# Ced3-han/PepFlowww

Hardware: AMD Instinct MI355X
Metric: residues x denoise-steps / s (higher is better)
Workload: dtype f32 (fp32 storage and accumulation; matrix products as 3 x f16 split MFMA, ~22-bit operands); 1 GPU; cfg4/GPU: B=64 x 128-residue synthetic pockets (112 ctx + 16 gen) per GPU; per_gpu_batch=64, residues=128, global_batch=64, parallelism=batch-shard x1, hipgraph=True, precision=fp32

## Files before the change

### pepflowww_amd/csrc/ipa_split.hip

```cpp
#include <cstdlib>
#include <type_traits>
#include "common.h"
#include "../../include/pepflow_hip.h"

#ifdef PF_PROFILE
__device__ long long g_prof_ipas[64];
#define PROFS(i) do { if (blockIdx.x == gridDim.x / 2 + 3 && threadIdx.x == 64) g_prof_ipas[i] = clock64(); } while (0)
extern "C" int pf_debug_prof_ipas(long long* out, int n) {
    return (int)hipMemcpyFromSymbol(out, HIP_SYMBOL(g_prof_ipas), sizeof(long long) * n, 0, hipMemcpyDeviceToHost);
}
#else
#define PROFS(i)
#endif

namespace {

typedef float f32x2 __attribute__((ext_vector_type(2)));
constexpr int H = PF_HEADS, C = PF_C_HID, PQ = PF_QK_PTS, PV = PF_V_PTS;
constexpr int OFF_KV = 1024;
#ifndef PF_IPA_WMAX
#define PF_IPA_WMAX 8
#endif
constexpr int WMAX = PF_IPA_WMAX;
constexpr int KPS = 28;
// ... 968 lines not shown
        }
    };
    half8 kh[4], nh[4];
    if constexpr (!PROJ) { if (wave_on) loadk(0, kh); }

    if constexpr (PROJ) {
        for (int j = tid; j < LK; j += blockDim.x) MJ[j] = a.mask[rowb + j];
        for (int idx = tid; idx < PF_ATT_VROWS * (L32 - LK); idx += blockDim.x) {
            const int row = idx / (L32 - LK), col = LK + idx - row * (L32 - LK);
            VT[row * VTS + col] = (_Float16)0.f;
        }
        unsigned char* WS = reinterpret_cast<unsigned char*>(SW);
        float* QPW = reinterpret_cast<float*>(WS + PJ16_STAGE_B) + wave * (1536 / 4);
        float* PB = reinterpret_cast<float*>(WS + PJ16_STAGE_B) + (blockDim.x >> 6) * (1536 / 4);
        proj_head16<KF>(a, rowb, wave_on ? iq : 0, h, i0 + r, wave_on, KP, KL, VT, VTS, WS, QPW, PB, qh, qp4, lane, wave, (int)(blockDim.x >> 6));
        __syncthreads();
        if (!wave_on) return;
        loadk(0, kh);
    } else {

    {
        const int nth = blockDim.x;
        constexpr int KB = 6;
        float4 k4[KB];
#pragma unroll
        for (int u = 0; u < KB; ++u) {
            const int idx = min(tid + u * nth, max(LK * 6 - 1, 0)), j = idx / 6, q = idx - j * 6;
            k4[u] = *reinterpret_cast<const float4*>(a.kp + (rowb + j) * 192 + h * 24 + 4 * q);
        }
        float mj0 = a.mask[rowb + min(tid, max(LK - 1, 0))];
        asm volatile("" : "+v"(k4[0].x), "+v"(k4[0].y), "+v"(k4[0].z), "+v"(k4[0].w), "+v"(k4[1].x), "+v"(k4[1].y), "+v"(k4[1].z), "+v"(k4[1].w),
                          "+v"(k4[2].x), "+v"(k4[2].y), "+v"(k4[2].z), "+v"(k4[2].w), "+v"(mj0));
        asm volatile("" : "+v"(k4[3].x), "+v"(k4[3].y), "+v"(k4[3].z), "+v"(k4[3].w), "+v"(k4[4].x), "+v"(k4[4].y), "+v"(k4[4].z), "+v"(k4[4].w),
                          "+v"(k4[5].x), "+v"(k4[5].y), "+v"(k4[5].z), "+v"(k4[5].w));
#pragma unroll
        for (int u = 0; u < KB; ++u) {
            const int idx = tid + u * nth, j = idx / 6, q = idx - j * 6;
            if (idx < LK * 6) *reinterpret_cast<float4*>(KP + j * KPS + 4 * q) = k4[u];
        }
        if (tid < LK) MJ[tid] = mj0;
        for (int idx = tid + KB * nth; idx < LK * 6; idx += nth) {
            const int j = idx / 6, q = idx - j * 6;
            *reinterpret_cast<float4*>(KP + j * KPS + 4 * q) = *reinterpret_cast<const float4*>(a.kp + (rowb + j) * 192 + h * 24 + 4 * q);
        }
        for (int j = tid + nth; j < LK; j += nth) MJ[j] = a.mask[rowb + j];
    }
    __syncthreads();
    if (!wave_on) return;
    }
    PROFS(1);

    const float scale_qk = 0.051031036307982884f;
    const float* brow = a.bias + (((size_t)b * H + h) * L + iq) * L;
    float* srow = SW + (size_t)wave * 16 * SLD + r * SLD;
    float mx = -3.0e38f;
    auto qk_tile = [&](int t, const half8 (&kh)[4], const float4& bv) {
        const int jb = 16 * t + 4 * g;
        const float bj[4] = {bv.x, bv.y, bv.z, bv.w};
        f32x4 am = {0.f, 0.f, 0.f, 0.f};
#pragma unroll
        for (int s4 = 0; s4 < 4; ++s4) am = mfma_h(kh[s4], qh[s4], am);
        float sv[4];
#pragma unroll
        for (int e = 0; e < 4; ++e) {
            const int j = jb + e;
            const float* kp = KP + j * KPS;
            f32x2 d2 = {0.f, 0.f};
#pragma unroll
            for (int q = 0; q < 6; ++q) {
                const float4 kq = *reinterpret_cast<const float4*>(kp + 4 * q);
                const f32x2 da = (f32x2){qp4[q].x, qp4[q].y} - (f32x2){kq.x, kq.y};
                const f32x2 db = (f32x2){qp4[q].z, qp4[q].w} - (f32x2){kq.z, kq.w};
                d2 = __builtin_elementwise_fma(da, da, d2);
                d2 = __builtin_elementwise_fma(db, db, d2);
            }
            float v = am[e] * scale_qk + bj[e];
            v = v + (-0.5f) * (gamma * (d2[0] + d2[1]));
            v = v + 1e5f * (mi * MJ[j] - 1.f);
            sv[e] = v;
            mx = fmaxf(mx, v);
        }
        *reinterpret_cast<float4*>(srow + jb) = make_float4(sv[0], sv[1], sv[2], sv[3]);
    };
    {
        float4 bc = *reinterpret_cast<const float4*>(brow + 4 * g), bn;
        int t = 0;
        for (; t + 1 < kt; t += 2) {
            loadk(t + 1, nh);
            bn = *reinterpret_cast<const float4*>(brow + 16 * (t + 1) + 4 * g);
            __builtin_amdgcn_sched_barrier(0);
            qk_tile(t, kh, bc);
            __builtin_amdgcn_sched_barrier(0);
            loadk(min(t + 2, kt - 1), kh);
            bc = *reinterpret_cast<const float4*>(brow + 16 * min(t + 2, kt - 1) + 4 * g);
            __builtin_amdgcn_sched_barrier(0);
            qk_tile(t + 1, nh, bn);
            __builtin_amdgcn_sched_barrier(0);
        }
        if (kt & 1) qk_tile(kt - 1, kh, bc);
    }
    PROFS(2);
    mx = max_xor32(max_xor16(mx));
    float sum = 0.f;
    for (int t = 0; t < kt; ++t) {
        float4 v = *reinterpret_cast<const float4*>(srow + 16 * t + 4 * g);
        v.x = exp_softmax(v.x - mx); v.y = exp_softmax(v.y - mx); v.z = exp_softmax(v.z - mx); v.w = exp_softmax(v.w - mx);
        sum += v.x; sum += v.y; sum += v.z; sum += v.w;
        *reinterpret_cast<float4*>(srow + 16 * t + 4 * g) = v;
    }
    if (L32 > LK) *reinterpret_cast<float4*>(srow + LK + 4 * g) = make_float4(0.f, 0.f, 0.f, 0.f);
    sum = sum_xor32(sum_xor16(sum));
    const float inv = 1.f / sum;
    asm volatile("s_waitcnt lgkmcnt(0)" ::: "memory");
    __builtin_amdgcn_wave_barrier();
    PROFS(3);
    if constexpr (FUSE) pair_dz_phase<true>(a, rowb, h, i0, LK, kt, SW + (size_t)wave * 16 * SLD, SLD, inv, lane);
    PROFS(7);
    float* prow = FUSE ? nullptr : a.p_out + (((size_t)b * H + h) * L + iq) * L;

    constexpr int NTC = 11;
    const _Float16* vt = reinterpret_cast<const _Float16*>(a.att_vt) + ((size_t)b * H + h) * PF_ATT_VT_HEAD(L);
    int vrow[NTC];
#pragma unroll
    for (int n = 0; n < NTC; ++n) vrow[n] = n < 8 ? 8 * r + n : min(128 + 16 * (n - 8) + r, PF_ATT_VROWS - 1);
    auto loadv = [&](int s32, half8 (&vh)[NTC]) {
#pragma unroll
        for (int n = 0; n < NTC; ++n) {
            if constexpr (PROJ) vh[n] = *reinterpret_cast<const half8*>(VT + vrow[n] * VTS + 32 * s32 + 8 * g);
            else vh[n] = *reinterpret_cast<const half8*>(vt + ((size_t)(n * PF_ATT_VT_NST(L) + s32) * 64 + lane) * 8);
        }
    };
    f32x4 Om[NTC];
#pragma unroll
    for (int n = 0; n < NTC; ++n) Om[n] = (f32x4){0.f, 0.f, 0.f, 0.f};
    const int ns = L32 >> 5;
    auto pv_step = [&](int s32, const half8 (&vh)[NTC]) {
        float4 p0 = *reinterpret_cast<const float4*>(srow + 32 * s32 + 8 * g);
        float4 p1 = *reinterpret_cast<const float4*>(srow + 32 * s32 + 8 * g + 4);
        p0.x *= inv; p0.y *= inv; p0.z *= inv; p0.w *= inv;
        p1.x *= inv; p1.y *= inv; p1.z *= inv; p1.w *= inv;
        if (!FUSE && 32 * s32 + 8 * g < LK) {
            *reinterpret_cast<float4*>(prow + 32 * s32 + 8 * g) = p0;
            *reinterpret_cast<float4*>(prow + 32 * s32 + 8 * g + 4) = p1;
        }
        half8 ph;
        ph[0] = (_Float16)p0.x; ph[1] = (_Float16)p0.y; ph[2] = (_Float16)p0.z; ph[3] = (_Float16)p0.w;
        ph[4] = (_Float16)p1.x; ph[5] = (_Float16)p1.y; ph[6] = (_Float16)p1.z; ph[7] = (_Float16)p1.w;
#pragma unroll
        for (int n = 0; n < NTC; ++n) Om[n] = mfma_h(ph, vh[n], Om[n]);
    };
    {
        half8 va[NTC], vb2[NTC];
        loadv(0, va);
        int s32 = 0;
        for (; s32 + 1 < ns; s32 += 2) {
            loadv(s32 + 1, vb2);
            __builtin_amdgcn_sched_barrier(0);
            pv_step(s32, va);
            __builtin_amdgcn_sched_barrier(0);
            loadv(min(s32 + 2, ns - 1), va);
            __builtin_amdgcn_sched_barrier(0);
            pv_step(s32 + 1, vb2);
            __builtin_amdgcn_sched_barrier(0);
        }
        if (ns & 1) pv_step(ns - 1, va);
    }
    PROFS(4);
    float* opt = SW + (size_t)wave * 16 * SLD;
    asm volatile("s_waitcnt lgkmcnt(0)" ::: "memory");
    __builtin_amdgcn_wave_barrier();
#pragma unroll
    for (int e = 0; e < 4; ++e) {
        const int ti = 4 * g + e, i = i0 + ti;
        float o[NTC];
#pragma unroll
        for (int n = 0; n < NTC; ++n) o[n] = Om[n][e];
        float* f = a.feats + (rowb + i) * PF_IPA_FEATS + h * C + 8 * r;
        *reinterpret_cast<float4*>(f) = make_float4(o[0], o[1], o[2], o[3]);
        *reinterpret_cast<float4*>(f + 4) = make_float4(o[4], o[5], o[6], o[7]);
        opt[ti * 36 + r] = o[8];
        opt[ti * 36 + 16 + r] = o[9];
        if (r < 4) opt[ti * 36 + 32 + r] = o[10];
    }
    asm volatile("s_waitcnt lgkmcnt(0)" ::: "memory");
    __builtin_amdgcn_wave_barrier();
    PROFS(5);
    for (int idx = lane; idx < 16 * PV; idx += 64) {
        const int ti = idx / PV, p = idx - ti * PV;
        const int i = i0 + ti;
        const float* R = a.rot + (rowb + i) * 9;
        const float* T = a.trans + (rowb + i) * 3;
        const float* o = opt + ti * 36 + p * 3;
        const float x = o[0] - T[0], y = o[1] - T[1], z = o[2] - T[2];
        const float lx = R[0] * x + R[3] * y + R[6] * z;
        const float ly = R[1] * x + R[4] * y + R[7] * z;
        const float lz = R[2] * x + R[5] * y + R[8] * z;
        float* f = a.feats + (rowb + i) * PF_IPA_FEATS + h * PV + p;
        f[1024] = lx;
        f[1120] = ly;
        f[1216] = lz;
        f[1312] = sqrtf(lx * lx + ly * ly + lz * lz + 1e-8f);
    }
    PROFS(6);
}

constexpr int ZW = 4;
template <int NG, bool Z16 = false>
__global__ __launch_bounds__(64 * ZW) void ipa_pair_kernel(pf_ipa_attn_args a) {
    constexpr int LPZ = 16 * NG;
    extern __shared__ __attribute__((aligned(16))) float smem[];
    const int tid = threadIdx.x, wave = tid >> 6, lane = tid & 63;
    const int r = lane & 15, g = lane >> 4;
    const int L = a.L;
    float* PL = smem;
    float* ZBAR = PL + 8 * LPZ;
    float* WL = ZBAR + ZW * 8 * 64;
    const long row = blockIdx.x;
    const long b = row / L, i = row - b * L;
    const int Le = a.key_end ? min(__builtin_amdgcn_readfirstlane(a.key_end[b]), L) : L;
    if (i >= Le) return;
    const int nge = (Le + 15) >> 4;
    const float* zrow = a.z + (size_t)row * L * 64 + 4 * r;
    const _Float16* zrow16 = reinterpret_cast<const _Float16*>(a.z) + (size_t)row * L * 64 + 4 * r;
    float4 zq[NG];
    half4 zq16[NG];
#pragma unroll
    for (int u = 0; u < NG; ++u) {
        const int j = 4 * (4 * u + wave) + g;
        if (u < nge) {
            if constexpr (Z16) zq16[u] = *reinterpret_cast<const half4*>(zrow16 + (size_t)min(j, L - 1) * 64);
            else zq[u] = *reinterpret_cast<const float4*>(zrow + (size_t)min(j, L - 1) * 64);
        }
    }
    const float4 wq4 = *reinterpret_cast<const float4*>(a.w_dz + r * 64 + 16 * g + 4 * wave);    const float bdz = a.b_dz[r];
    if ((L & 3) == 0) {
        for (int idx = tid; idx < LPZ * 2; idx += 64 * ZW) {
            const int hh = idx / (LPZ / 4), j = 4 * (idx - hh * (LPZ / 4));
            float4 v = make_float4(0.f, 0.f, 0.f, 0.f);
            if (j < Le) {
                v = *reinterpret_cast<const float4*>(a.p_out + ((b * H + hh) * L + i) * L + j);
                if (j + 1 >= Le) v.y = 0.f;
                if (j + 2 >= Le) v.z = 0.f;
                if (j + 3 >= Le) v.w = 0.f;
            }
            *reinterpret_cast<float4*>(PL + hh * LPZ + j) = v;
        }
    } else {
        for (int idx = tid; idx < LPZ * 8; idx += 64 * ZW) {
            const int hh = idx / LPZ, j = idx - hh * LPZ;
            PL[idx] = j < Le ? a.p_out[((b * H + hh) * L + i) * L + j] : 0.f;
        }
    }
    *reinterpret_cast<float4*>(WL + (wave * 64 + lane) * 4) = wq4;
    __syncthreads();
    f32x4 zacc[4];
#pragma unroll
    for (int ct = 0; ct < 4; ++ct) zacc[ct] = (f32x4){0.f, 0.f, 0.f, 0.f};
    const float* pl = PL + (r & 7) * LPZ + g;
    const float keep = r < 8 ? 1.f : 0.f;
#pragma unroll
    for (int u = 0; u < NG; ++u) {
        if (u < nge) {
            const float pa = pl[4 * (4 * u + wave)] * keep;
            if constexpr (Z16) zq[u] = make_float4((float)zq16[u][0], (float)zq16[u][1], (float)zq16[u][2], (float)zq16[u][3]);
            zacc[0] = mfma16(pa, zq[u].x, zacc[0]);
            zacc[1] = mfma16(pa, zq[u].y, zacc[1]);
            zacc[2] = mfma16(pa, zq[u].z, zacc[2]);
            zacc[3] = mfma16(pa, zq[u].w, zacc[3]);
        }
    }
    if (g < 2) {
        float* zb = ZBAR + wave * H * 64;
#pragma unroll
        for (int e = 0; e < 4; ++e)
            *reinterpret_cast<float4*>(zb + (4 * g + e) * 64 + 4 * r) = make_float4(zacc[0][e], zacc[1][e], zacc[2][e], zacc[3][e]);
    }
    __syncthreads();
    if (wave == 0) {
        f32x4 oacc[4];
#pragma unroll
        for (int q = 0; q < 4; ++q) oacc[q] = (f32x4){0.f, 0.f, 0.f, 0.f};
        float wdz[16];
#pragma unroll
        for (int q = 0; q < 4; ++q) {
            const float4 w4 = *reinterpret_cast<const float4*>(WL + (q * 64 + lane) * 4);
            wdz[4 * q] = w4.x; wdz[4 * q + 1] = w4.y; wdz[4 * q + 2] = w4.z; wdz[4 * q + 3] = w4.w;
        }
        const float* zs = ZBAR + (r & 7) * 64 + 16 * g;
#pragma unroll
        for (int s4 = 0; s4 < 16; ++s4) {
            float za = zs[s4];
#pragma unroll
            for (int q = 1; q < ZW; ++q) za += zs[q * H * 64 + s4];
            oacc[s4 & 3] = mfma16(za * keep, wdz[s4], oacc[s4 & 3]);
        }
        if (g < 2) {
#pragma unroll
            for (int e = 0; e < 4; ++e)
                a.feats[(size_t)row * PF_IPA_FEATS + 1408 + (4 * g + e) * 16 + r] = ((oacc[0][e] + oacc[1][e]) + (oacc[2][e] + oacc[3][e])) + bdz;
        }
    }
}

template <int NG, bool D16 = false>
__global__ __launch_bounds__(256) void ipa_pair_dz_kernel(pf_ipa_attn_args a) {
    constexpr int LPZ = 16 * NG;
    extern __shared__ __attribute__((aligned(16))) float smem[];
    const int tid = threadIdx.x, wave = tid >> 6, lane = tid & 63;
    const int r = lane & 15, g = lane >> 4;
    const int L = a.L;
    const long row = (long)blockIdx.x * 4 + wave;
    if (row >= (long)a.B * L) return;
    const long b = row / L, i = row - b * L;
    const int Le = a.key_end ? min(__builtin_amdgcn_readfirstlane(a.key_end[b]), L) : L;
    if (i >= Le) return;
    const int nge = (Le + 15) >> 4;
    float* PL = smem + wave * 8 * LPZ;
    const float* drow = a.dz + (size_t)row * L * 16 + r;
    const _Float16* drow16 = reinterpret_cast<const _Float16*>(a.dz) + (size_t)row * L * 16 + r;
    float bv[NG][4];
    _Float16 bv16[NG][4];
#pragma unroll
    for (int u = 0; u < NG; ++u)
        if (u < nge) {
#pragma unroll
            for (int t = 0; t < 4; ++t) {
                const size_t off = (size_t)min(16 * u + 4 * t + g, L - 1) * 16;
                if constexpr (D16) bv16[u][t] = drow16[off];
                else bv[u][t] = drow[off];
            }
        }
    const float bdz = a.b_dz[r];
    if ((L & 3) == 0) {
        for (int idx = lane; idx < LPZ * 2; idx += 64) {
            const int hh = idx / (LPZ / 4), j = 4 * (idx - hh * (LPZ / 4));
            float4 v = make_float4(0.f, 0.f, 0.f, 0.f);
            if (j < Le) {
                v = *reinterpret_cast<const float4*>(a.p_out + ((b * H + hh) * L + i) * L + j);
                if (j + 1 >= Le) v.y = 0.f;
                if (j + 2 >= Le) v.z = 0.f;
                if (j + 3 >= Le) v.w = 0.f;
            }
            float* d = PL + hh * LPZ + (j & ~15) + ((j >> 2) & 3);
            d[0] = v.x; d[4] = v.y; d[8] = v.z; d[12] = v.w;
        }
    } else {
        for (int idx = lane; idx < LPZ * 8; idx += 64) {
            const int hh = idx / LPZ, j = idx - hh * LPZ;
            PL[hh * LPZ + (j & ~15) + 4 * (j & 3) + ((j >> 2) & 3)] = j < Le ? a.p_out[((b * H + hh) * L + i) * L + j] : 0.f;
        }
    }
    asm volatile("s_waitcnt lgkmcnt(0)" ::: "memory");
    __builtin_amdgcn_wave_barrier();
    f32x4 acc[4];
#pragma unroll
    for (int t = 0; t < 4; ++t) acc[t] = (f32x4){0.f, 0.f, 0.f, 0.f};
    const float* pl = PL + (r & 7) * LPZ + 4 * g;
    const float keep = r < 8 ? 1.f : 0.f;
#pragma unroll
    for (int u = 0; u < NG; ++u) {
        if (u < nge) {
            const float4 pa = *reinterpret_cast<const float4*>(pl + 16 * u);
            if constexpr (D16) {
#pragma unroll
                for (int t = 0; t < 4; ++t) bv[u][t] = (float)bv16[u][t];
            }
            acc[0] = mfma16(pa.x * keep, bv[u][0], acc[0]);
            acc[1] = mfma16(pa.y * keep, bv[u][1], acc[1]);
            acc[2] = mfma16(pa.z * keep, bv[u][2], acc[2]);
            acc[3] = mfma16(pa.w * keep, bv[u][3], acc[3]);
        }
    }
    if (g < 2) {
        float* f = a.feats + (size_t)row * PF_IPA_FEATS + 1408 + r;
#pragma unroll
        for (int e = 0; e < 4; ++e) f[(4 * g + e) * 16] = ((acc[0][e] + acc[1][e]) + (acc[2][e] + acc[3][e])) + bdz;
    }
}

template <int NG>
__global__ __launch_bounds__(256) void ipa_pair_dz16_kernel(pf_ipa_attn_args a) {
    constexpr int LPZ = 16 * NG;
    extern __shared__ __attribute__((aligned(16))) float smem[];
    const int tid = threadIdx.x, wave = tid >> 6, lane = tid & 63;
    const int ks = (lane & 3) | ((lane >> 4) << 2), q = (lane >> 2) & 3;
    const int L = a.L;
    const long row = (long)blockIdx.x * 4 + wave;
    if (row >= (long)a.B * L) return;
    const long b = row / L, i = row - b * L;
    const int Le = a.key_end ? min(__builtin_amdgcn_readfirstlane(a.key_end[b]), L) : L;
    if (i >= Le) return;
    const int nge = (Le + 15) >> 4;
    float* PL = smem + wave * 8 * LPZ;
    const _Float16* drow = reinterpret_cast<const _Float16*>(a.dz) + (size_t)row * L * 16 + 4 * q;
    half4 d[NG];
#pragma unroll
    for (int u = 0; u < NG; ++u)
        if (u < nge) d[u] = *reinterpret_cast<const half4*>(drow + (size_t)min(16 * u + ks, L - 1) * 16);
    if ((L & 3) == 0) {
        for (int idx = lane; idx < LPZ * 2; idx += 64) {
            const int hh = idx / (LPZ / 4), j = 4 * (idx - hh * (LPZ / 4));
            float4 v = make_float4(0.f, 0.f, 0.f, 0.f);
            if (j < Le) {
                v = *reinterpret_cast<const float4*>(a.p_out + ((b * H + hh) * L + i) * L + j);
                if (j + 1 >= Le) v.y = 0.f;
                if (j + 2 >= Le) v.z = 0.f;
                if (j + 3 >= Le) v.w = 0.f;
            }
            *reinterpret_cast<float4*>(PL + hh * LPZ + j) = v;
        }
    } else {
        for (int idx = lane; idx < LPZ * 8; idx += 64) {
            const int hh = idx / LPZ, j = idx - hh * LPZ;
            PL[idx] = j < Le ? a.p_out[((b * H + hh) * L + i) * L + j] : 0.f;
        }
    }
    asm volatile("s_waitcnt lgkmcnt(0)" ::: "memory");
    __builtin_amdgcn_wave_barrier();
    float v[32];
#pragma unroll
    for (int k = 0; k < 32; ++k) v[k] = 0.f;
#pragma unroll
    for (int u = 0; u < NG; ++u) {
        if (u < nge) {
            const float d0 = (float)d[u][0], d1 = (float)d[u][1], d2 = (float)d[u][2], d3 = (float)d[u][3];
#pragma unroll
            for (int h = 0; h < 8; ++h) {
                const float ph = PL[h * LPZ + 16 * u + ks];
                v[4 * h] += ph * d0; v[4 * h + 1] += ph * d1; v[4 * h + 2] += ph * d2; v[4 * h + 3] += ph * d3;
            }
        }
    }
    float w[16], x[8], y[4], z2[2];
    {
        const bool hi = lane & 1;
#pragma unroll
        for (int k = 0; k < 16; ++k) {
            const float send = hi ? v[k] : v[k + 16], keep = hi ? v[k + 16] : v[k];
            w[k] = keep + lane_xor1(send);
        }
    }
    {
        const bool hi = lane & 2;
#pragma unroll
        for (int k = 0; k < 8; ++k) {
            const float send = hi ? w[k] : w[k + 8], keep = hi ? w[k + 8] : w[k];
            x[k] = keep + lane_xor2(send);
        }
    }
#pragma unroll
    for (int k = 0; k < 4; ++k) {
        auto rr = __builtin_amdgcn_permlane16_swap(__float_as_uint(x[k]), __float_as_uint(x[k + 4]), false, false);
        y[k] = __uint_as_float(rr[0]) + __uint_as_float(rr[1]);
    }
#pragma unroll
    for (int k = 0; k < 2; ++k) {
        auto rr = __builtin_amdgcn_permlane32_swap(__float_as_uint(y[k]), __float_as_uint(y[k + 2]), false, false);
        z2[k] = __uint_as_float(rr[0]) + __uint_as_float(rr[1]);
    }
    const int h = ((lane & 1) << 2) | (lane & 2) | ((lane >> 4) & 1), c = 4 * q + 2 * (lane >> 5);
    const float2 bd = *reinterpret_cast<const float2*>(a.b_dz + c);
    *reinterpret_cast<float2*>(a.feats + (size_t)row * PF_IPA_FEATS + 1408 + h * 16 + c) = make_float2(z2[0] + bd.x, z2[1] + bd.y);
}

}

extern "C" int pf_ipa_proj_inside_ok(int L, int f16_mode) {
    if (L < 1) return 0;
    const int LP = (L + 15) & ~15, SLD = LP + 4 < 36 ? 36 : LP + 4, tiles = LP >> 4;
    if (f16_mode) {
        if ((L & 15) != 0 || tiles > WMAX) return 0;
        const int L32 = (L + 31) & ~31, SLD16 = L32 + 4 < 36 ? 36 : L32 + 4;
        const size_t fixed16 = ((size_t)L * KPS + L) * sizeof(float);
        const size_t swb = (size_t)tiles * 16 * SLD16 * sizeof(float), stg = (size_t)PJ16_STAGE_B + (size_t)tiles * 1536 + (size_t)PJ_TILES * 64;
        const size_t lds16 = fixed16 + (swb > stg ? swb : stg) + ((size_t)L * KLS + (size_t)PF_ATT_VROWS * (L32 + 8)) * sizeof(_Float16);
        return lds16 <= 160 * 1024;
    }
    if ((L & 3) != 0) return 0;
    const size_t fixed = ((size_t)LP * KPS + LP + (size_t)pj_vp_floats(LP)) * sizeof(float), per_wave = (size_t)16 * SLD * sizeof(float);
    if (fixed + per_wave > 160 * 1024) return 0;
    int wmax = (int)((160 * 1024 - fixed) / per_wave);
    wmax = wmax > WMAX ? WMAX : wmax;
    if (tiles > WMAX && tiles % WMAX != 0 && wmax > 4) wmax = 4;
    if (wmax < 1) return 0;
    const int nrb = (tiles + wmax - 1) / wmax, wpb = (tiles + nrb - 1) / nrb;
    if (nrb != 1) return 0;
    const size_t lds = fixed + wpb * per_wave;
    const size_t need = fixed + (size_t)PJ_STAGE_B + (size_t)wpb * 16 * 24 * sizeof(float) + (size_t)PJ_TILES * 16 * sizeof(float);
    return (lds > need ? lds : need) <= 160 * 1024;
}

int pf_ipa_split_launch(const pf_ipa_attn_args* a, hipStream_t s) {
    const int L = a->L;
    int rc = 0;
    const bool pj16 = a->s_in && a->att_mode == 2 && (L & 15) == 0;
    if (a->k_from_s && !a->s_in) return PF_E_BADARG;
    if (a->att_mode == 1) return PF_E_BADARG;
    const bool planes = ((a->att_qk && a->att_vt) || pj16) && a->att_mode == 2 && (L & 15) == 0;
    const bool fuse = a->fused_pair && a->dz && (planes ? a->dz_f16 != 0 : a->dz_f16 == 0);
    if (!fuse && !a->p_out) return PF_E_BADARG;
    {
        const int LP = (L + 15) & ~15, SLD = LP + 4 < 36 ? 36 : LP + 4;
        const int tiles = LP >> 4;
        const bool pj = a->s_in != nullptr && !pj16;
        const size_t fixed = ((size_t)LP * KPS + LP + (size_t)(pj ? pj_vp_floats(LP) : LP * VPS)) * sizeof(float), per_wave = (size_t)16 * SLD * sizeof(float);
        int wmax = (int)((160 * 1024 - fixed) / per_wave);
        wmax = wmax > WMAX ? WMAX : wmax;
        if (tiles > WMAX && tiles % WMAX != 0 && wmax > 4) wmax = 4;
        if (wmax < 1) return PF_E_TOOLARGE;
        const int nrb = (tiles + wmax - 1) / wmax;
        const int wpb = (tiles + nrb - 1) / nrb;
        const size_t lds = fixed + wpb * per_wave;
        static PfOncePerDevice attr_set;
        if (attr_set.first()) {
            (void)hipFuncSetAttribute((const void*)ipa_scores_kernel<true>, hipFuncAttributeMaxDynamicSharedMemorySize, 160 * 1024);
            (void)hipFuncSetAttribute((const void*)ipa_scores_kernel<false>, hipFuncAttributeMaxDynamicSharedMemorySize, 160 * 1024);
            (void)hipFuncSetAttribute((const void*)ipa_scores_kernel<true, true>, hipFuncAttributeMaxDynamicSharedMemorySize, 160 * 1024);
            (void)hipFuncSetAttribute((const void*)ipa_scores_kernel<false, true>, hipFuncAttributeMaxDynamicSharedMemorySize, 160 * 1024);
            (void)hipFuncSetAttribute((const void*)ipa_scores_kernel<true, false, false, true>, hipFuncAttributeMaxDynamicSharedMemorySize, 160 * 1024);
            (void)hipFuncSetAttribute((const void*)ipa_scores_kernel<true, true, false, true>, hipFuncAttributeMaxDynamicSharedMemorySize, 160 * 1024);
        }
        if (pj16) {
            if (tiles > WMAX || !a->proj_w_f16 || !a->proj_bias || !fuse) return PF_E_BADARG;
            const int L32 = (L + 31) & ~31, SLD16 = L32 + 4 < 36 ? 36 : L32 + 4;
            const size_t fixed16 = ((size_t)L * KPS + L) * sizeof(float);
            const size_t swb = (size_t)tiles * 16 * SLD16 * sizeof(float), stg = (size_t)PJ16_STAGE_B + (size_t)tiles * 1536 + (size_t)PJ_TILES * 64;
            const size_t lds16 = fixed16 + (swb > stg ? swb : stg) + ((size_t)L * KLS + (size_t)PF_ATT_VROWS * (L32 + 8)) * sizeof(_Float16);
            if (lds16 > 160 * 1024) return PF_E_TOOLARGE;
            static PfOncePerDevice attr_pj16;
            if (attr_pj16.first()) {
                (void)hipFuncSetAttribute((const void*)ipa_scores16_kernel<true, true>, hipFuncAttributeMaxDynamicSharedMemorySize, 160 * 1024);
                (void)hipFuncSetAttribute((const void*)ipa_scores16_kernel<true, true, true>, hipFuncAttributeMaxDynamicSharedMemorySize, 160 * 1024);
            }
            if (a->k_from_s) hipLaunchKernelGGL((ipa_scores16_kernel<true, true, true>), dim3((unsigned)(a->B * H)), dim3(64 * tiles), lds16, s, *a, 1, 16 * tiles, SLD16);
            else hipLaunchKernelGGL((ipa_scores16_kernel<true, true>), dim3((unsigned)(a->B * H)), dim3(64 * tiles), lds16, s, *a, 1, 16 * tiles, SLD16);
            PF_CHECK_LAUNCH();
            return 0;
        }
        if (a->k_frag && (a->s_in || planes || (L & 15) != 0)) return PF_E_BADARG;
        if (pj && (planes || nrb != 1 || (L & 3) != 0 || !a->proj_w_f16 || !a->proj_bias || !a->proj || !a->att_vt || a->ldp < OFF_KV + 2 * H * C)) return PF_E_BADARG;
        if (pj) {
            static PfOncePerDevice attr_pj;
            if (attr_pj.first()) {
                (void)hipFuncSetAttribute((const void*)ipa_scores_kernel<true, false, true, false, false, true>, hipFuncAttributeMaxDynamicSharedMemorySize, 160 * 1024);
                (void)hipFuncSetAttribute((const void*)ipa_scores_kernel<true, true, true, false, false, true>, hipFuncAttributeMaxDynamicSharedMemorySize, 160 * 1024);
                (void)hipFuncSetAttribute((const void*)ipa_scores_kernel<true, false, true, false, true, true>, hipFuncAttributeMaxDynamicSharedMemorySize, 160 * 1024);
                (void)hipFuncSetAttribute((const void*)ipa_scores_kernel<true, true, true, false, true, true>, hipFuncAttributeMaxDynamicSharedMemorySize, 160 * 1024);
                (void)hipFuncSetAttribute((const void*)ipa_scores_kernel<true, false, true, false, false, false>, hipFuncAttributeMaxDynamicSharedMemorySize, 160 * 1024);
                (void)hipFuncSetAttribute((const void*)ipa_scores_kernel<true, true, true, false, false, false>, hipFuncAttributeMaxDynamicSharedMemorySize, 160 * 1024);
                (void)hipFuncSetAttribute((const void*)ipa_scores_kernel<true, false, true, false, true, false>, hipFuncAttributeMaxDynamicSharedMemorySize, 160 * 1024);
                (void)hipFuncSetAttribute((const void*)ipa_scores_kernel<true, true, true, false, true, false>, hipFuncAttributeMaxDynamicSharedMemorySize, 160 * 1024);
            }
            const size_t need = fixed + (size_t)PJ_STAGE_B + (size_t)wpb * 16 * 24 * sizeof(float) + (size_t)PJ_TILES * 16 * sizeof(float);
            const size_t ldsp = lds > need ? lds : need;
            if (ldsp > 160 * 1024) return PF_E_TOOLARGE;
            const int nwv = wpb <= 4 ? 2 * wpb : wpb;
#define PF_SCORES_PJ(FUSEv, KFv) do { \
                if (nwv != wpb) hipLaunchKernelGGL((ipa_scores_kernel<true, FUSEv, true, false, KFv, true>), dim3((unsigned)(a->B * H * nrb)), dim3(64 * nwv), ldsp, s, *a, nrb, 16 * wpb, LP, SLD); \
                else hipLaunchKernelGGL((ipa_scores_kernel<true, FUSEv, true, false, KFv, false>), dim3((unsigned)(a->B * H * nrb)), dim3(64 * nwv), ldsp, s, *a, nrb, 16 * wpb, LP, SLD); } while (0)
            if (a->k_from_s) {
                if (fuse) PF_SCORES_PJ(true, true);
                else PF_SCORES_PJ(false, true);
            } else if (fuse) PF_SCORES_PJ(true, false);
            else PF_SCORES_PJ(false, false);
#undef PF_SCORES_PJ
        } else if (planes) {
            const int L32 = (L + 31) & ~31, SLD16 = L32 + 4 < 36 ? 36 : L32 + 4;
            const size_t fixed16 = ((size_t)L * KPS + L) * sizeof(float), pw16 = (size_t)16 * SLD16 * sizeof(float);
            int wm = (int)((160 * 1024 - fixed16) / pw16);
            wm = wm > WMAX ? WMAX : wm;
            if (tiles > WMAX && tiles % WMAX != 0 && wm > 4) wm = 4;
            if (tiles <= 4 && wm > 2) wm = 2;
            if (wm < 1) return PF_E_TOOLARGE;
            const int nrb16 = (tiles + wm - 1) / wm, wpb16 = (tiles + nrb16 - 1) / nrb16;
            const size_t lds16 = fixed16 + wpb16 * pw16;
            static PfOncePerDevice attr16;
            if (attr16.first()) {
                (void)hipFuncSetAttribute((const void*)ipa_scores16_kernel<false>, hipFuncAttributeMaxDynamicSharedMemorySize, 160 * 1024);
                (void)hipFuncSetAttribute((const void*)ipa_scores16_kernel<true>, hipFuncAttributeMaxDynamicSharedMemorySize, 160 * 1024);
            }
            const dim3 g16((unsigned)(a->B * H * nrb16)), b16(64 * wpb16);
            if (fuse) hipLaunchKernelGGL((ipa_scores16_kernel<true>), g16, b16, lds16, s, *a, nrb16, 16 * wpb16, SLD16);
            else hipLaunchKernelGGL(ipa_scores16_kernel<false>, g16, b16, lds16, s, *a, nrb16, 16 * wpb16, SLD16);
        } else if (a->k_frag) {
            if (fuse) hipLaunchKernelGGL((ipa_scores_kernel<true, true, false, true>), dim3((unsigned)(a->B * H * nrb)), dim3(64 * wpb), lds, s, *a, nrb, 16 * wpb, LP, SLD);
            else hipLaunchKernelGGL((ipa_scores_kernel<true, false, false, true>), dim3((unsigned)(a->B * H * nrb)), dim3(64 * wpb), lds, s, *a, nrb, 16 * wpb, LP, SLD);
        } else if (fuse) {
            if ((L & 3) == 0) hipLaunchKernelGGL((ipa_scores_kernel<true, true>), dim3((unsigned)(a->B * H * nrb)), dim3(64 * wpb), lds, s, *a, nrb, 16 * wpb, LP, SLD);
            else hipLaunchKernelGGL((ipa_scores_kernel<false, true>), dim3((unsigned)(a->B * H * nrb)), dim3(64 * wpb), lds, s, *a, nrb, 16 * wpb, LP, SLD);
        } else if ((L & 3) == 0)
            hipLaunchKernelGGL(ipa_scores_kernel<true>, dim3((unsigned)(a->B * H * nrb)), dim3(64 * wpb), lds, s, *a, nrb, 16 * wpb, LP, SLD);
        else
            hipLaunchKernelGGL(ipa_scores_kernel<false>, dim3((unsigned)(a->B * H * nrb)), dim3(64 * wpb), lds, s, *a, nrb, 16 * wpb, LP, SLD);
        PF_CHECK_LAUNCH();
    }
    if (rc) return rc;
    if (fuse) return 0;
    const int ng = (L + 15) / 16;
    const size_t lds = ((size_t)8 * 16 * ng + ZW * 8 * 64 + 4 * 64 * 4) * sizeof(float);
    const long rows = (long)a->B * L;
    if (ng > 16 || rows > 0x7fffffffL) return PF_E_TOOLARGE;
    if (a->dz) {
        const dim3 gridd((unsigned)((rows + 3) / 4));
        const size_t ldsd = (size_t)4 * 8 * 16 * ng * sizeof(float);
        switch (ng) {
#define PF_PAIRDZ_CASE(N) case N: if (a->dz_f16) hipLaunchKernelGGL(ipa_pair_dz16_kernel<N>, gridd, dim3(256), ldsd, s, *a); else hipLaunchKernelGGL((ipa_pair_dz_kernel<N, false>), gridd, dim3(256), ldsd, s, *a); break;
            PF_PAIRDZ_CASE(1) PF_PAIRDZ_CASE(2) PF_PAIRDZ_CASE(3) PF_PAIRDZ_CASE(4) PF_PAIRDZ_CASE(5) PF_PAIRDZ_CASE(6) PF_PAIRDZ_CASE(7)
            PF_PAIRDZ_CASE(8) PF_PAIRDZ_CASE(9) PF_PAIRDZ_CASE(10) PF_PAIRDZ_CASE(11) PF_PAIRDZ_CASE(12) PF_PAIRDZ_CASE(13)
            PF_PAIRDZ_CASE(14) PF_PAIRDZ_CASE(15) PF_PAIRDZ_CASE(16)
#undef PF_PAIRDZ_CASE
        }
        PF_CHECK_LAUNCH();
        return 0;
    }
    const dim3 grid((unsigned)rows), blk(64 * ZW);
    switch (ng) {
#define PF_PAIR_CASE(N) case N: if (a->z_f16) hipLaunchKernelGGL((ipa_pair_kernel<N, true>), grid, blk, lds, s, *a); else hipLaunchKernelGGL(ipa_pair_kernel<N>, grid, blk, lds, s, *a); break;
        PF_PAIR_CASE(1) PF_PAIR_CASE(2) PF_PAIR_CASE(3) PF_PAIR_CASE(4) PF_PAIR_CASE(5) PF_PAIR_CASE(6) PF_PAIR_CASE(7) PF_PAIR_CASE(8)
        PF_PAIR_CASE(9) PF_PAIR_CASE(10) PF_PAIR_CASE(11) PF_PAIR_CASE(12) PF_PAIR_CASE(13) PF_PAIR_CASE(14) PF_PAIR_CASE(15) PF_PAIR_CASE(16)
#undef PF_PAIR_CASE
    }
    PF_CHECK_LAUNCH();
    return 0;
}
```

Measured before the change: 2.927 million res*step/s.

## Restructure fp32 pair-dz kernel with bucketed unroll, padded LDS and occupancy bounds

Rewrites the fp32 ipa_pair_dz kernel around a helper that is instantiated for a compile-time number of key groups. A recursive picker selects the smallest instantiation (in steps of two) covering the actual key extent, replacing runtime `u < nge` guards. It also issues the p_out float4 loads before the dz loads to overlap latency, and pads and swizzles the LDS row stride to reduce bank conflicts. It adds occupancy hints to launch_bounds and uses 32-bit offsets, at the cost of more template instantiations and code size. This path only runs when dz is not fp16.

After: 2.963 million res*step/s (median of 6 runs). +1.2%, better.

```diff
diff --git a/pepflowww_amd/csrc/ipa_split.hip b/pepflowww_amd/csrc/ipa_split.hip
--- a/pepflowww_amd/csrc/ipa_split.hip
+++ b/pepflowww_amd/csrc/ipa_split.hip
@@ -1294,80 +1294,105 @@
     }
 }
 
+__device__ __forceinline__ int pdz_slot(int u, int g) { return 16 * u + 4 * ((g + (u >> 1)) & 3); }
+
+template <class T> __device__ __forceinline__ T ld_boff(const void* base, unsigned byte_off) { return *reinterpret_cast<const T*>(reinterpret_cast<const char*>(base) + byte_off); }
+
+template <int NG, int NU, bool D16, bool V4>
+__device__ __forceinline__ void pair_dz_row(const pf_ipa_attn_args& a, float* PL, long row, long b, long i, int Le, int lane) {
+    constexpr int LPU = 16 * NU, LDP = 16 * NG + 8, NP = (2 * LPU + 63) / 64;
+    const int r = lane & 15, g = lane >> 4;
+    const int L = a.L;
+    float4 pv[NP];
+    const float* prow = a.p_out + ((size_t)b * H * L + i) * L;
+    if constexpr (V4) {
+#pragma unroll
+        for (int k = 0; k < NP; ++k) {
+            const int idx = lane + 64 * k, hh = min(idx / (LPU / 4), H - 1), j = 4 * (idx % (LPU / 4));
+            pv[k] = ld_boff<float4>(prow, 4u * (unsigned)(hh * L * L + (j < Le ? j : 0)));
+        }
+    }
+    const float* drow = a.dz + (size_t)row * L * 16;
+    const _Float16* drow16 = reinterpret_cast<const _Float16*>(a.dz) + (size_t)row * L * 16;
+    float bv[NU][4];
+    _Float16 bv16[NU][4];
+#pragma unroll
+    for (int u = 0; u < NU; ++u) {
+#pragma unroll
+        for (int t = 0; t < 4; ++t) {
+            const unsigned off = (unsigned)min(16 * u + 4 * t + g, Le - 1) * 16u + r;
+            if constexpr (D16) bv16[u][t] = ld_boff<_Float16>(drow16, 2u * off);
+            else bv[u][t] = ld_boff<float>(drow, 4u * off);
+        }
+    }
+    const float bdz = a.b_dz[r];
+    if constexpr (V4) {
+#pragma unroll
+        for (int k = 0; k < NP; ++k) {
+            const int idx = lane + 64 * k, hh = idx / (LPU / 4), j = 4 * (idx % (LPU / 4));
+            if (2 * LPU % 64 == 0 || idx < 2 * LPU) {
+                const float4 v = pv[k];
+                float* d = PL + hh * LDP + ((j >> 2) & 3);
+                const int u = j >> 4;
+                d[pdz_slot(u, 0)] = j < Le ? v.x : 0.f;
+                d[pdz_slot(u, 1)] = j + 1 < Le ? v.y : 0.f;
+                d[pdz_slot(u, 2)] = j + 2 < Le ? v.z : 0.f;
+                d[pdz_slot(u, 3)] = j + 3 < Le ? v.w : 0.f;
+            }
+        }
+    } else {
+        for (int idx = lane; idx < LPU * 8; idx += 64) {
+            const int hh = idx / LPU, j = idx - hh * LPU;
+            PL[hh * LDP + pdz_slot(j >> 4, j & 3) + ((j >> 2) & 3)] = j < Le ? ld_boff<float>(prow, 4u * (unsigned)(hh * L * L + j)) : 0.f;
+        }
+    }
+    asm volatile("s_waitcnt lgkmcnt(0)" ::: "memory");
+    __builtin_amdgcn_wave_barrier();
+    f32x4 acc[4];
+#pragma unroll
+    for (int t = 0; t < 4; ++t) acc[t] = (f32x4){0.f, 0.f, 0.f, 0.f};
+    const float* pl = PL + (r & 7) * LDP;
+#pragma unroll
+    for (int u = 0; u < NU; ++u) {
+        const float4 pa = *reinterpret_cast<const float4*>(pl + pdz_slot(u, g));
+        if constexpr (D16) {
+#pragma unroll
+            for (int t = 0; t < 4; ++t) bv[u][t] = (float)bv16[u][t];
+        }
+        acc[0] = mfma16(pa.x, bv[u][0], acc[0]);
+        acc[1] = mfma16(pa.y, bv[u][1], acc[1]);
+        acc[2] = mfma16(pa.z, bv[u][2], acc[2]);
+        acc[3] = mfma16(pa.w, bv[u][3], acc[3]);
+    }
+    if (g < 2) {
+        float* f = a.feats + (size_t)row * PF_IPA_FEATS + 1408;
+#pragma unroll
+        for (int e = 0; e < 4; ++e) f[(unsigned)((4 * g + e) * 16 + r)] = ((acc[0][e] + acc[1][e]) + (acc[2][e] + acc[3][e])) + bdz;
+    }
+}
+
+template <int NG, int NU, bool D16, bool V4>
+__device__ __forceinline__ void pair_dz_pick(const pf_ipa_attn_args& a, float* PL, long row, long b, long i, int Le, int nge, int lane) {
+    if constexpr (NU <= 2) pair_dz_row<NG, NU, D16, V4>(a, PL, row, b, i, Le, lane);
+    else {
+        if (nge > NU - 2) pair_dz_row<NG, NU, D16, V4>(a, PL, row, b, i, Le, lane);
+        else pair_dz_pick<NG, NU - 2, D16, V4>(a, PL, row, b, i, Le, nge, lane);
+    }
+}
+
 template <int NG, bool D16 = false>
-__global__ __launch_bounds__(256) void ipa_pair_dz_kernel(pf_ipa_attn_args a) {
-    constexpr int LPZ = 16 * NG;
+__global__ __launch_bounds__(256, NG <= 8 ? 8 : NG <= 11 ? 5 : 4) void ipa_pair_dz_kernel(pf_ipa_attn_args a) {
     extern __shared__ __attribute__((aligned(16))) float smem[];
-    const int tid = threadIdx.x, wave = tid >> 6, lane = tid & 63;
-    const int r = lane & 15, g = lane >> 4;
+    const int tid = threadIdx.x, wave = __builtin_amdgcn_readfirstlane(tid >> 6), lane = tid & 63;
     const int L = a.L;
     const long row = (long)blockIdx.x * 4 + wave;
     if (row >= (long)a.B * L) return;
-    const long b = row / L, i = row - b * L;
+    const long b = (unsigned)row / (unsigned)L, i = row - b * L;
     const int Le = a.key_end ? min(__builtin_amdgcn_readfirstlane(a.key_end[b]), L) : L;
     if (i >= Le) return;
-    const int nge = (Le + 15) >> 4;
-    float* PL = smem + wave * 8 * LPZ;
-    const float* drow = a.dz + (size_t)row * L * 16 + r;
-    const _Float16* drow16 = reinterpret_cast<const _Float16*>(a.dz) + (size_t)row * L * 16 + r;
-    float bv[NG][4];
-    _Float16 bv16[NG][4];
-#pragma unroll
-    for (int u = 0; u < NG; ++u)
-        if (u < nge) {
-#pragma unroll
-            for (int t = 0; t < 4; ++t) {
-                const size_t off = (size_t)min(16 * u + 4 * t + g, L - 1) * 16;
-                if constexpr (D16) bv16[u][t] = drow16[off];
-                else bv[u][t] = drow[off];
-            }
-        }
-    const float bdz = a.b_dz[r];
-    if ((L & 3) == 0) {
-        for (int idx = lane; idx < LPZ * 2; idx += 64) {
-            const int hh = idx / (LPZ / 4), j = 4 * (idx - hh * (LPZ / 4));
-            float4 v = make_float4(0.f, 0.f, 0.f, 0.f);
-            if (j < Le) {
-                v = *reinterpret_cast<const float4*>(a.p_out + ((b * H + hh) * L + i) * L + j);
-                if (j + 1 >= Le) v.y = 0.f;
-                if (j + 2 >= Le) v.z = 0.f;
-                if (j + 3 >= Le) v.w = 0.f;
-            }
-            float* d = PL + hh * LPZ + (j & ~15) + ((j >> 2) & 3);
-            d[0] = v.x; d[4] = v.y; d[8] = v.z; d[12] = v.w;
-        }
-    } else {
-        for (int idx = lane; idx < LPZ * 8; idx += 64) {
-            const int hh = idx / LPZ, j = idx - hh * LPZ;
-            PL[hh * LPZ + (j & ~15) + 4 * (j & 3) + ((j >> 2) & 3)] = j < Le ? a.p_out[((b * H + hh) * L + i) * L + j] : 0.f;
-        }
-    }
-    asm volatile("s_waitcnt lgkmcnt(0)" ::: "memory");
-    __builtin_amdgcn_wave_barrier();
-    f32x4 acc[4];
-#pragma unroll
-    for (int t = 0; t < 4; ++t) acc[t] = (f32x4){0.f, 0.f, 0.f, 0.f};
-    const float* pl = PL + (r & 7) * LPZ + 4 * g;
-    const float keep = r < 8 ? 1.f : 0.f;
-#pragma unroll
-    for (int u = 0; u < NG; ++u) {
-        if (u < nge) {
-            const float4 pa = *reinterpret_cast<const float4*>(pl + 16 * u);
-            if constexpr (D16) {
-#pragma unroll
-                for (int t = 0; t < 4; ++t) bv[u][t] = (float)bv16[u][t];
-            }
-            acc[0] = mfma16(pa.x * keep, bv[u][0], acc[0]);
-            acc[1] = mfma16(pa.y * keep, bv[u][1], acc[1]);
-            acc[2] = mfma16(pa.z * keep, bv[u][2], acc[2]);
-            acc[3] = mfma16(pa.w * keep, bv[u][3], acc[3]);
-        }
-    }
-    if (g < 2) {
-        float* f = a.feats + (size_t)row * PF_IPA_FEATS + 1408 + r;
-#pragma unroll
-        for (int e = 0; e < 4; ++e) f[(4 * g + e) * 16] = ((acc[0][e] + acc[1][e]) + (acc[2][e] + acc[3][e])) + bdz;
-    }
+    float* PL = smem + wave * 8 * (16 * NG + 8);
+    if ((L & 3) == 0) pair_dz_pick<NG, NG, D16, true>(a, PL, row, b, i, Le, (Le + 15) >> 4, lane);
+    else pair_dz_pick<NG, NG, D16, false>(a, PL, row, b, i, Le, (Le + 15) >> 4, lane);
 }
 
 template <int NG>
@@ -1594,7 +1619,7 @@
     if (ng > 16 || rows > 0x7fffffffL) return PF_E_TOOLARGE;
     if (a->dz) {
         const dim3 gridd((unsigned)((rows + 3) / 4));
-        const size_t ldsd = (size_t)4 * 8 * 16 * ng * sizeof(float);
+        const size_t ldsd = (size_t)4 * 8 * (a->dz_f16 ? 16 * ng : 16 * ng + 8) * sizeof(float);
         switch (ng) {
 #define PF_PAIRDZ_CASE(N) case N: if (a->dz_f16) hipLaunchKernelGGL(ipa_pair_dz16_kernel<N>, gridd, dim3(256), ldsd, s, *a); else hipLaunchKernelGGL((ipa_pair_dz_kernel<N, false>), gridd, dim3(256), ldsd, s, *a); break;
             PF_PAIRDZ_CASE(1) PF_PAIRDZ_CASE(2) PF_PAIRDZ_CASE(3) PF_PAIRDZ_CASE(4) PF_PAIRDZ_CASE(5) PF_PAIRDZ_CASE(6) PF_PAIRDZ_CASE(7)
```
